# evfro/polara

Measured on NVIDIA H100. Metric: user-item pairs scored/sec (fused top-k) at rank 50, higher is better.
Workload: dtype f32 (bf16 tensor-core filter, exact fp32 rescoring)

## Files before the change

polara_b200/csrc/topk_tc.cu:

```cuda
#include <cuda_bf16.h>
#include <cstdlib>
#include <cub/device/device_radix_sort.cuh>

#include "topk_common.cuh"

namespace {

constexpr int BM = 128;
constexpr int BN = 128;
constexpr int NCONS = 256;
constexpr int NTHREADS = NCONS + 32;
constexpr int CAPS = 16;
constexpr int MAX_STAGES = 10;
constexpr uint32_t STAGE_BYTES = BN * 128;
constexpr int PROBE_ITEMS = 256;
constexpr int HEAD_TILES = 8;
constexpr int HEAD_WORDS = HEAD_TILES * BN / 32;
constexpr long long SPIN_LIMIT_CYCLES = 4000000000ll;

struct TcParams {
    const __nv_bfloat16* Ap;
    const __nv_bfloat16* Bp;
    const float* E; int64_t lde;
    const float* V; int64_t ldv;
// ... 106 lines not shown

__device__ __forceinline__ uint32_t bf16_floor_bits(float x) {
    uint32_t b = __float_as_uint(x);
    uint32_t hi = b >> 16;
    if ((b & 0xFFFFu) && (b >> 31)) hi += 1;
    return hi;
}
__device__ __forceinline__ uint32_t bf16_ceil_pos_bits(float x) {
    uint32_t b = __float_as_uint(x);
    return (b >> 16) + ((b & 0xFFFFu) ? 1u : 0u);
}
__device__ __forceinline__ uint32_t pack_threshold(float t) {
    if (!(t > -3.0e38f)) t = -3.0e38f;
    t -= fabsf(t) * 1.52587890625e-5f;
    uint32_t hi = bf16_floor_bits(t);
    float hif = __uint_as_float(hi << 16);
    float rem = t - hif;
    uint32_t lo = bf16_floor_bits(rem);
    return (lo << 16) | (hi & 0xFFFFu);
}

__global__ void pack_items_kernel(const float* __restrict__ V, int64_t ldv, int64_t n, int r, int rs, int KP,
                                  int64_t item_tiles, const int32_t* __restrict__ perm,
                                  const float* __restrict__ vnorm_sorted, __nv_bfloat16* __restrict__ Bp) {
    const int chunks = (KP + 63) / 64 * 8;
    int64_t gid = (int64_t)blockIdx.x * blockDim.x + threadIdx.x;
    int64_t total = item_tiles * BN * chunks;
    if (gid >= total) return;
    int64_t tile = gid / ((int64_t)BN * chunks);
    int rem = (int)(gid % ((int64_t)BN * chunks));
    int row = rem / chunks, ch = rem % chunks;
    int64_t pos = tile * BN + row;
    const int64_t item = pos < n ? (int64_t)__ldg(perm + pos) : -1;
    __align__(16) __nv_bfloat16 out[8];
#pragma unroll
    for (int j = 0; j < 8; ++j) {
        int kk = ch * 8 + j;
        float x = 0.f;
        if (item >= 0) {
            if (kk < r) x = __ldg(V + item * ldv + kk);
            else if (kk == rs || kk == rs + 1) x = 1.0f;
        }
        out[j] = __float2bfloat16_rn(x);
        if (item >= 0 && kk == rs + 2) out[j] = __ushort_as_bfloat16((unsigned short)bf16_ceil_pos_bits(__ldg(vnorm_sorted + pos)));
    }
    size_t byte = (size_t)tile * BN * chunks * 16 + tile_byte(BN, row, ch * 8);
    *reinterpret_cast<uint4*>(reinterpret_cast<unsigned char*>(Bp) + byte) = *reinterpret_cast<const uint4*>(out);
}

__global__ void pack_users_kernel(const float* __restrict__ E, int64_t lde, int64_t m, int r, int rs, int KP,
                                  int64_t user_tiles, const int32_t* __restrict__ uperm, const float* __restrict__ enorm,
                                  const float* __restrict__ t0, __nv_bfloat16* __restrict__ Ap) {
    const int chunks = (KP + 63) / 64 * 8;
    int64_t gid = (int64_t)blockIdx.x * blockDim.x + threadIdx.x;
    int64_t total = user_tiles * BM * chunks;
    if (gid >= total) return;
    int64_t tile = gid / ((int64_t)BM * chunks);
    int rem = (int)(gid % ((int64_t)BM * chunks));
    int row = rem / chunks, ch = rem % chunks;
    const int64_t tr = tile * BM + row;
    const int64_t u = (tr < m && uperm) ? (int64_t)__ldg(uperm + tr) : tr;
    __align__(16) __nv_bfloat16 out[8];
    uint32_t thr = 0;
    if (ch == rs / 8) {
        if (u < m) {
            thr = pack_threshold(t0[u]);
        } else {
            thr = 0x00007F7Fu;
        }
    }
#pragma unroll
    for (int j = 0; j < 8; ++j) {
        int kk = ch * 8 + j;
        float x = 0.f;
        if (u < m && kk < r) x = -__ldg(E + u * lde + kk);
        out[j] = __float2bfloat16_rn(x);
        if (kk == rs) out[j] = __ushort_as_bfloat16((unsigned short)(thr & 0xFFFFu));
        if (kk == rs + 1) out[j] = __ushort_as_bfloat16((unsigned short)(thr >> 16));
        if (kk == rs + 2 && u < m)
            out[j] = __ushort_as_bfloat16((unsigned short)(0x8000u | bf16_ceil_pos_bits(0.0079345703125f * enorm[u] + 1e-30f)));
    }
    size_t byte = (size_t)tile * BM * chunks * 16 + tile_byte(BM, row, ch * 8);
    *reinterpret_cast<uint4*>(reinterpret_cast<unsigned char*>(Ap) + byte) = *reinterpret_cast<const uint4*>(out);
}

__global__ void row_norm_kernel(const float* __restrict__ X, int64_t ld, int64_t rows, int r, float* __restrict__ norms,
                                float* __restrict__ max_out) {
    int64_t w = ((int64_t)blockIdx.x * blockDim.x + threadIdx.x) >> 5;
    int lane = threadIdx.x & 31;
    if (w >= rows) return;
    float s = 0.f;
    for (int t = lane; t < r; t += 32) { float x = __ldg(X + w * ld + t); s = fmaf(x, x, s); }
#pragma unroll
    for (int o = 16; o > 0; o >>= 1) s += __shfl_xor_sync(0xffffffffu, s, o);
    s = sqrtf(s) * 1.0001f;
    if (lane == 0) {
        if (norms) norms[w] = s;
        if (max_out) atomicMax(reinterpret_cast<int*>(max_out), __float_as_int(s));
    }
}

__global__ void iota_i32_kernel(int32_t* __restrict__ x, int64_t n) {
    int64_t i = (int64_t)blockIdx.x * blockDim.x + threadIdx.x;
    if (i < n) x[i] = (int32_t)i;
}

__global__ void invert_perm_kernel(const int32_t* __restrict__ perm, int64_t n, int32_t* __restrict__ inv) {
    int64_t i = (int64_t)blockIdx.x * blockDim.x + threadIdx.x;
    if (i < n) inv[perm[i]] = (int32_t)i;
}

__global__ void head_items_kernel(const int32_t* __restrict__ perm, int64_t n_head, uint32_t* __restrict__ in_head) {
    int64_t i = (int64_t)blockIdx.x * blockDim.x + threadIdx.x;
    if (i < n_head) { const int32_t item = perm[i]; atomicOr(in_head + (item >> 5), 1u << (item & 31)); }
}

__global__ void __launch_bounds__(256)
head_bitmap_kernel(const int64_t* __restrict__ seen_indptr, const int32_t* __restrict__ seen_indices,
                   int64_t seen_offset, const int32_t* __restrict__ inv_perm, const uint32_t* __restrict__ in_head,
                   int64_t m, int64_t n, uint32_t* __restrict__ bits) {
    static_assert(HEAD_WORDS == 32, "one bitmap word per lane");
    __shared__ uint32_t sw[8][HEAD_WORDS];
    const int64_t u = ((int64_t)blockIdx.x * blockDim.x + threadIdx.x) >> 5;
    const int lane = threadIdx.x & 31, warp = threadIdx.x >> 5;
    if (u >= m) return;
    sw[warp][lane] = 0u;
    __syncwarp();
    for (int64_t p = seen_indptr[u] + lane; p < seen_indptr[u + 1]; p += 32) {
        int64_t item = (int64_t)__ldg(seen_indices + p) - seen_offset;
        if (item < 0 || item >= n) continue;
        if (!((__ldg(in_head + (item >> 5)) >> (item & 31)) & 1u)) continue;
        int pos = __ldg(inv_perm + item);
        atomicOr(&sw[warp][pos >> 5], 0x80000000u >> (pos & 31));
    }
    __syncwarp();
    bits[u * HEAD_WORDS + lane] = sw[warp][lane];
}

__device__ __forceinline__ int first_cut_tile(float en, float t, const float* __restrict__ vnorm_sorted, int lo, int hi) {
    if (!(t > 0.f && t < CUDART_INF_F)) return hi;
    while (lo < hi) {
        const int mid = (lo + hi) >> 1;
        if (en * __ldg(vnorm_sorted + (int64_t)mid * BN) < t) hi = mid; else lo = mid + 1;
    }
    return lo;
}

__global__ void user_need_kernel(const float* __restrict__ enorm, const float* __restrict__ t0,
                                 const float* __restrict__ vnorm_sorted, int64_t m, int item_tiles, int32_t* __restrict__ need) {
    const int64_t u = (int64_t)blockIdx.x * blockDim.x + threadIdx.x;
    if (u < m) need[u] = first_cut_tile(__ldg(enorm + u), __ldg(t0 + u), vnorm_sorted, 0, item_tiles);
}

constexpr int PTU = 64, PTI = 128, PKS = 32;
constexpr int PNU = 2;
template <int PI>
struct ProbeSmem {
    float es[PKS][PTU + 4];
    float vs[PKS][PTI + 4];
    float sc[PTU][PI + 4];
    unsigned long long cand[8][PNU][32];
    float t0s[PTU];
};

__device__ __forceinline__ uint32_t ord_of(float x) {
    const uint32_t b = __float_as_uint(x);
    return (b & 0x80000000u) ? ~b : (b | 0x80000000u);
}
__device__ __forceinline__ float ord_to_float(uint32_t o) {
    return __uint_as_float((o & 0x80000000u) ? (o & 0x7FFFFFFFu) : ~o);
}

template <int PL>
__device__ __noinline__ void probe_select_rounds(unsigned long long (&key)[PL], int lane, int k,
                                                 pb200_cand* __restrict__ out, float* __restrict__ t0_u) {
    static_assert(PL == 8, "the sorting network below is for 8 keys per lane");
#define PB_CAS(A, B) { const unsigned long long x_ = key[A], y_ = key[B]; const bool g_ = x_ > y_; key[A] = g_ ? x_ : y_; key[B] = g_ ? y_ : x_; }
    PB_CAS(0, 1) PB_CAS(2, 3) PB_CAS(4, 5) PB_CAS(6, 7)
    PB_CAS(0, 2) PB_CAS(1, 3) PB_CAS(4, 6) PB_CAS(5, 7)
    PB_CAS(1, 2) PB_CAS(5, 6)
    PB_CAS(0, 4) PB_CAS(1, 5) PB_CAS(2, 6) PB_CAS(3, 7)
    PB_CAS(2, 4) PB_CAS(3, 5)
    PB_CAS(1, 2) PB_CAS(3, 4) PB_CAS(5, 6)
#undef PB_CAS
    float kth = -CUDART_INF_F;
    int produced = 0;
    pb200_cand mine; mine.score = -CUDART_INF_F; mine.id = -1;
    for (; produced < k; ++produced) {
        const uint32_t hh = (uint32_t)(key[0] >> 32), hl = (uint32_t)key[0];
        const uint32_t wh = __reduce_max_sync(0xffffffffu, hh);
        if (wh == 0u) break;
        const uint32_t wl = __reduce_max_sync(0xffffffffu, hh == wh ? hl : 0u);
        if (hh == wh && hl == wl) {
#pragma unroll
            for (int j = 0; j + 1 < PL; ++j) key[j] = key[j + 1];
            key[PL - 1] = 0ull;
        }
        const float ws = ord_to_float(wh);
        if (lane == (produced & 31)) { mine.score = ws; mine.id = (int)(0xFFFFFFFFu - wl); }
        if ((produced & 31) == 31) out[(produced - 31) + lane] = mine;
        kth = ws;
    }
    if (lane < (produced & 31)) out[(produced & ~31) + lane] = mine;
    for (int j = produced + lane; j < k; j += 32) { pb200_cand c; c.score = -CUDART_INF_F; c.id = -1; out[j] = c; }
    if (lane == 0) *t0_u = produced == k ? kth : -CUDART_INF_F;
}

template <int PI>
__global__ void __launch_bounds__(256)
probe_kernel(const float* __restrict__ E, int64_t lde, const float* __restrict__ V, int64_t ldv,
             const int32_t* __restrict__ perm, int64_t m, int64_t n_probe, int r, int k,
             const uint32_t* __restrict__ headbits, float* __restrict__ t0, pb200_cand* __restrict__ out_list,
             float* __restrict__ enorm, const float* __restrict__ vnorm_sorted, int item_tiles, int32_t* __restrict__ need) {
    extern __shared__ __align__(16) unsigned char praw[];
    ProbeSmem<PI>& sm = *reinterpret_cast<ProbeSmem<PI>*>(praw);
    const int tid = threadIdx.x, lane = tid & 31, warp = tid >> 5, tx = tid & 15, ty = tid >> 4;
    const int64_t u0 = (int64_t)blockIdx.x * PTU;
    const bool vec = ((lde | ldv) & 3) == 0 && ((reinterpret_cast<uintptr_t>(E) | reinterpret_cast<uintptr_t>(V)) & 15) == 0;
    const int n_ktiles = (r + PKS - 1) / PKS, n_tiles = (PI / PTI) * n_ktiles;
    const int64_t eu = u0 + (tid & (PTU - 1));
    const float* erow = eu < m ? E + eu * lde : nullptr;
    const float* vrow = nullptr;
    float4 pe[2], pv[4];
    auto fetch = [&](int tile) {
        const int i0 = (tile / n_ktiles) * PTI, k0 = (tile % n_ktiles) * PKS;
        if (tile % n_ktiles == 0) {
            const int64_t vpos = i0 + (tid & (PTI - 1));
            vrow = vpos < n_probe ? V + (int64_t)__ldg(perm + vpos) * ldv : nullptr;
        }
#pragma unroll
        for (int it = 0; it < 2; ++it) {
            const int kq = k0 + 4 * ((tid >> 6) + 4 * it);
            pe[it] = (erow && kq < r) ? __ldg(reinterpret_cast<const float4*>(erow + kq)) : make_float4(0.f, 0.f, 0.f, 0.f);
        }
#pragma unroll
        for (int it = 0; it < 4; ++it) {
            const int kq = k0 + 4 * ((tid >> 7) + 2 * it);
            pv[it] = (vrow && kq < r) ? __ldg(reinterpret_cast<const float4*>(vrow + kq)) : make_float4(0.f, 0.f, 0.f, 0.f);
        }
    };
    auto stash = [&](int tile) {
        const int k0 = (tile % n_ktiles) * PKS;
#pragma unroll
        for (int it = 0; it < 2; ++it) {
            const int q = (tid >> 6) + 4 * it, kq = k0 + 4 * q, row = tid & (PTU - 1);
            sm.es[4 * q + 0][row] = pe[it].x;
            sm.es[4 * q + 1][row] = kq + 1 < r ? pe[it].y : 0.f;
            sm.es[4 * q + 2][row] = kq + 2 < r ? pe[it].z : 0.f;
            sm.es[4 * q + 3][row] = kq + 3 < r ? pe[it].w : 0.f;
        }
#pragma unroll
        for (int it = 0; it < 4; ++it) {
            const int q = (tid >> 7) + 2 * it, kq = k0 + 4 * q, row = tid & (PTI - 1);
            sm.vs[4 * q + 0][row] = pv[it].x;
            sm.vs[4 * q + 1][row] = kq + 1 < r ? pv[it].y : 0.f;
            sm.vs[4 * q + 2][row] = kq + 2 < r ? pv[it].z : 0.f;
            sm.vs[4 * q + 3][row] = kq + 3 < r ? pv[it].w : 0.f;
        }
    };
    if (vec) fetch(0);
    float acc[4][8];
    float en2 = 0.f;
    for (int tile = 0; tile < n_tiles; ++tile) {
        const int i0 = (tile / n_ktiles) * PTI, k0 = (tile % n_ktiles) * PKS;
        if (k0 == 0) {
#pragma unroll
            for (int a = 0; a < 4; ++a)
#pragma unroll
                for (int b = 0; b < 8; ++b) acc[a][b] = 0.f;
        }
        if (vec) {
            stash(tile);
        } else {
#pragma unroll
            for (int it = 0; it < 8; ++it) {
                int e = tid + it * 256, row = e >> 5, kk = e & 31;
                int64_t u = u0 + row;
                sm.es[kk][row] = (u < m && k0 + kk < r) ? __ldg(E + u * lde + k0 + kk) : 0.f;
            }
#pragma unroll
            for (int it = 0; it < 16; ++it) {
                int e = tid + it * 256, row = e >> 5, kk = e & 31;
                int64_t pos = i0 + row;
                sm.vs[kk][row] = (pos < n_probe && k0 + kk < r) ? __ldg(V + (int64_t)__ldg(perm + pos) * ldv + k0 + kk) : 0.f;
            }
        }
        __syncthreads();
        if (vec && tile + 1 < n_tiles) fetch(tile + 1);
        const int kmax = min(PKS, r - k0);
        if (i0 == 0 && tid < PTU)
            for (int kk = 0; kk < kmax; ++kk) en2 = fmaf(sm.es[kk][tid], sm.es[kk][tid], en2);
        for (int kk = 0; kk < kmax; ++kk) {
            float4 e4 = *reinterpret_cast<const float4*>(&sm.es[kk][ty * 4]);
            float4 v0 = *reinterpret_cast<const float4*>(&sm.vs[kk][tx * 4]);
            float4 v1 = *reinterpret_cast<const float4*>(&sm.vs[kk][64 + tx * 4]);
            float a[4] = {e4.x, e4.y, e4.z, e4.w};
            float b[8] = {v0.x, v0.y, v0.z, v0.w, v1.x, v1.y, v1.z, v1.w};
#pragma unroll
            for (int i = 0; i < 4; ++i)
#pragma unroll
                for (int j = 0; j < 8; ++j) acc[i][j] = fmaf(a[i], b[j], acc[i][j]);
        }
        if (k0 + PKS >= r) {
#pragma unroll
            for (int i = 0; i < 4; ++i)
#pragma unroll
                for (int hseg = 0; hseg < 2; ++hseg) {
                    const int pos = i0 + 64 * hseg + tx * 4;
                    float4 x;
                    x.x = pos + 0 < n_probe ? acc[i][4 * hseg + 0] : -CUDART_INF_F;
                    x.y = pos + 1 < n_probe ? acc[i][4 * hseg + 1] : -CUDART_INF_F;
                    x.z = pos + 2 < n_probe ? acc[i][4 * hseg + 2] : -CUDART_INF_F;
                    x.w = pos + 3 < n_probe ? acc[i][4 * hseg + 3] : -CUDART_INF_F;
                    *reinterpret_cast<float4*>(&sm.sc[ty * 4 + i][pos]) = x;
                }
        }
        __syncthreads();
    }
    constexpr int PL = PI / 32;
    const uint32_t lt_mask = (1u << lane) - 1u;
    for (int ul = warp; ul < PTU; ul += 8 * PNU) {
        int64_t u[PNU];
        bool act[PNU];
        uint32_t seen_w[PNU], ord[PNU][PL], lmax[PNU], tau[PNU];
        int count[PNU] = {};
#pragma unroll
        for (int a = 0; a < PNU; ++a) {
            u[a] = u0 + ul + 8 * a;
            act[a] = ul + 8 * a < PTU && u[a] < m;
            seen_w[a] = 0u;
            if (act[a] && headbits && lane < PL) seen_w[a] = __ldg(headbits + u[a] * HEAD_WORDS + lane);
        }
#pragma unroll
        for (int a = 0; a < PNU; ++a) {
            lmax[a] = 0u;
#pragma unroll
            for (int j = 0; j < PL; ++j) {
                const int pos = lane + 32 * j;
                const uint32_t w = __shfl_sync(0xffffffffu, seen_w[a], j);
                const bool ok = act[a] && pos < n_probe && !(w & (0x80000000u >> lane));
                ord[a][j] = ok ? ord_of(sm.sc[act[a] ? ul + 8 * a : 0][pos]) : 0u;
                lmax[a] = max(lmax[a], ord[a][j]);
            }
        }
        const bool small_k = k <= 32;
        if (small_k) {
            uint32_t rest[PNU], w[PNU];
#pragma unroll
            for (int a = 0; a < PNU; ++a) { rest[a] = lmax[a]; w[a] = 0u; }
            for (int i = 0; i < k; ++i) {
#pragma unroll
                for (int a = 0; a < PNU; ++a) {
                    w[a] = __reduce_max_sync(0xffffffffu, rest[a]);
                    if (rest[a] == w[a]) rest[a] = 0u;
                }
            }
#pragma unroll
            for (int a = 0; a < PNU; ++a) tau[a] = w[a] == 0u ? 1u : w[a];
#pragma unroll
            for (int a = 0; a < PNU; ++a) count[a] = 0;
#pragma unroll
            for (int j = 0; j < PL; ++j)
#pragma unroll
                for (int a = 0; a < PNU; ++a) {
                    const bool in = ord[a][j] >= tau[a];
                    const uint32_t b = __ballot_sync(0xffffffffu, in);
                    const int slot = count[a] + __popc(b & lt_mask);
                    if (in && slot < 32) sm.cand[warp][a][slot] = ((unsigned long long)ord[a][j] << 32) | (uint32_t)(lane + 32 * j);
                    count[a] += __popc(b);
                }
        }
        bool fast[PNU];
#pragma unroll
        for (int a = 0; a < PNU; ++a) fast[a] = act[a] && small_k && count[a] <= 32;
        __syncwarp();
        unsigned long long mine[PNU];
#pragma unroll
        for (int a = 0; a < PNU; ++a) {
            mine[a] = 0ull;
            if (fast[a] && lane < count[a]) {
                const unsigned long long c = sm.cand[warp][a][lane];
                const uint32_t id = (uint32_t)__ldg(perm + (uint32_t)c);
                mine[a] = (c & 0xFFFFFFFF00000000ull) | (unsigned long long)(0xFFFFFFFFu - id);
            }
        }
        __syncwarp();
#pragma unroll
        for (int a = 0; a < PNU; ++a) if (fast[a]) sm.cand[warp][a][lane] = mine[a];
        __syncwarp();
#pragma unroll
        for (int a = 0; a < PNU; ++a) {
            if (!fast[a]) continue;
            pb200_cand* out = out_list + u[a] * k;
            int rank = 0;
            for (int t = 0; t < count[a]; ++t) rank += sm.cand[warp][a][t] > mine[a] ? 1 : 0;
            if (lane < count[a] && rank < k) {
                pb200_cand c; c.score = ord_to_float((uint32_t)(mine[a] >> 32)); c.id = (int)(0xFFFFFFFFu - (uint32_t)mine[a]);
                out[rank] = c;
                if (rank == k - 1) sm.t0s[ul + 8 * a] = c.score;
            }
            if (count[a] < k) {
                if (lane >= count[a] && lane < k) { pb200_cand c; c.score = -CUDART_INF_F; c.id = -1; out[lane] = c; }
                if (lane == 0) sm.t0s[ul + 8 * a] = -CUDART_INF_F;
            }
        }
        __syncwarp();
#pragma unroll
        for (int a = 0; a < PNU; ++a) {
            if (!act[a] || fast[a]) continue;
            unsigned long long key[PL];
#pragma unroll
            for (int j = 0; j < PL; ++j) {
                const uint32_t id = ord[a][j] ? (uint32_t)__ldg(perm + lane + 32 * j) : 0u;
                key[j] = ord[a][j] ? (((unsigned long long)ord[a][j] << 32) | (unsigned long long)(0xFFFFFFFFu - id)) : 0ull;
            }
            probe_select_rounds<PL>(key, lane, k, out_list + u[a] * k, &sm.t0s[ul + 8 * a]);
        }
    }
    __syncthreads();
    if (tid < PTU && u0 + tid < m) {
        const int64_t uu = u0 + tid;
        const float t = sm.t0s[tid], en = sqrtf(en2) * 1.0001f;
        t0[uu] = t;
        enorm[uu] = en;
        if (need) need[uu] = first_cut_tile(en, t, vnorm_sorted, 0, item_tiles);
    }
}

__device__ __forceinline__ float exact_score_vec(const float* __restrict__ erow, const float* __restrict__ vrow, int r, bool vec_ok) {
    if (!vec_ok) return exact_score(erow, vrow, r);
    const int r4 = r / 4;
    const float4* e4 = reinterpret_cast<const float4*>(erow);
    const float4* v4 = reinterpret_cast<const float4*>(vrow);
    float s = 0.f;
    int t = 0;
    for (; t + 8 <= r4; t += 8) {
        float4 a[8], b[8];
#pragma unroll
        for (int i = 0; i < 8; ++i) { a[i] = __ldg(e4 + t + i); b[i] = __ldg(v4 + t + i); }
#pragma unroll
        for (int i = 0; i < 8; ++i) {
            s = fmaf(a[i].x, b[i].x, s); s = fmaf(a[i].y, b[i].y, s);
            s = fmaf(a[i].z, b[i].z, s); s = fmaf(a[i].w, b[i].w, s);
        }
    }
    for (; t + 4 <= r4; t += 4) {
        float4 a[4], b[4];
#pragma unroll
        for (int i = 0; i < 4; ++i) { a[i] = __ldg(e4 + t + i); b[i] = __ldg(v4 + t + i); }
#pragma unroll
        for (int i = 0; i < 4; ++i) {
            s = fmaf(a[i].x, b[i].x, s); s = fmaf(a[i].y, b[i].y, s);
            s = fmaf(a[i].z, b[i].z, s); s = fmaf(a[i].w, b[i].w, s);
        }
    }
    for (; t < r4; ++t) {
        float4 a = __ldg(e4 + t), b = __ldg(v4 + t);
        s = fmaf(a.x, b.x, s); s = fmaf(a.y, b.y, s); s = fmaf(a.z, b.z, s); s = fmaf(a.w, b.w, s);
    }
    for (int tt = r4 * 4; tt < r; ++tt) s = fmaf(__ldg(erow + tt), __ldg(vrow + tt), s);
    return s;
}

struct ListState {
    pb200_cand* list;
    int cnt;
    float kth;
};

__device__ __forceinline__ void list_insert(ListState& ls, int k, float s, int id) {
    if (ls.cnt == k) {
        pb200_cand last = ls.list[k - 1];
        if (!cand_before(s, id, last.score, last.id)) return;
    }
    int i = ls.cnt < k ? ls.cnt : k - 1;
    while (i > 0) {
        pb200_cand p = ls.list[i - 1];
        if (!cand_before(s, id, p.score, p.id)) break;
        ls.list[i] = p;
        --i;
    }
    pb200_cand c; c.score = s; c.id = id;
    ls.list[i] = c;
    if (ls.cnt < k) ls.cnt++;
    if (ls.cnt == k) ls.kth = ls.list[k - 1].score;
}

constexpr int COOP_MIN = 64;
struct CoopArgs {
    const float* V; int64_t ldv; const int32_t* perm; const int32_t* seen_indices; int64_t seen_offset; int64_t n; int r, k;
};
__device__ __noinline__ int coop_flush_row(const CoopArgs p, const float* __restrict__ erow, const uint2* __restrict__ stage_row,
                                           int n_entries, int64_t t_lo, int64_t sb, int64_t se, bool head_masked,
                                           pb200_cand* __restrict__ list, float t_row, bool vec_ok, int lane, int& cnt, float& kth) {
    int n_scored = 0;
    for (int e = 0; e < n_entries; ++e) {
        const uint2 ent = stage_row[e * 256];
        const int64_t pos = (int64_t)(t_lo + (ent.x >> 2)) * BN + (ent.x & 3) * 32 + lane;
        bool ok = ((ent.y << lane) & 0x80000000u) != 0u && pos < p.n;
        int item = -1;
        float s = 0.f;
        if (ok) {
            item = __ldg(p.perm + pos);
            if (sb < se && (!head_masked || pos >= HEAD_TILES * BN) &&
                seen_lookup(p.seen_indices, sb, se, (int)(item + p.seen_offset))) ok = false;
        }
        if (ok) {
            s = exact_score_vec(erow, p.V + (int64_t)item * p.ldv, p.r, vec_ok);
            ++n_scored;
            ok = !(s < t_row);
        }
        uint32_t pass = __ballot_sync(0xffffffffu, ok);
        while (pass) {
            const int l = __ffs(pass) - 1;
            pass &= pass - 1;
            const float sl = __shfl_sync(0xffffffffu, s, l);
            const int il = __shfl_sync(0xffffffffu, item, l);
            if (sl < t_row) continue;
            cnt = warp_list_insert(list, p.k, cnt, sl, il, lane);
            if (cnt == p.k) { kth = list[p.k - 1].score; t_row = fmaxf(t_row, kth); }
        }
    }
    return n_scored;
}

__global__ void __launch_bounds__(NTHREADS, 1)
score_topk_tc_kernel(const TcParams p) {
    extern __shared__ __align__(1024) unsigned char smem[];
    unsigned char* sA = smem + ((1024u - (smem_u32(smem) & 1023u)) & 1023u);
    unsigned char* sB = sA + p.a_bytes;
    uint2* sStage = reinterpret_cast<uint2*>(sB + (size_t)p.stages * STAGE_BYTES);
    volatile uint2* sThr = reinterpret_cast<volatile uint2*>(sStage + CAPS * 256);
    uint64_t* bars = reinterpret_cast<uint64_t*>(const_cast<uint2*>(sThr) + 256);
    const uint32_t bar_full = smem_u32(bars), bar_empty = smem_u32(bars + MAX_STAGES);
    const uint32_t bar_afull = smem_u32(bars + 2 * MAX_STAGES), bar_aempty = smem_u32(bars + 2 * MAX_STAGES + 1);
    volatile uint32_t* flush_gen = reinterpret_cast<volatile uint32_t*>(bars + 2 * MAX_STAGES + 2);
    volatile unsigned long long* sCut = reinterpret_cast<volatile unsigned long long*>(bars + 2 * MAX_STAGES + 4);
    volatile uint32_t* sStop = reinterpret_cast<volatile uint32_t*>(bars + 2 * MAX_STAGES + 4 + NCONS / 32);

    const int tid = threadIdx.x, warp = tid >> 5, lane = tid & 31;
    if (tid < 256) { const_cast<uint2*>(sThr)[tid] = make_uint2(0u, 0u); }
    if (tid < NCONS / 32) sCut[tid] = 0ull;
    if (tid < MAX_STAGES) sStop[tid] = 0u;
    if (tid == 0) {
        *flush_gen = 0u;
        for (int s = 0; s < p.stages; ++s) { mbar_init(bar_full + 8 * s, 1); mbar_init(bar_empty + 8 * s, NCONS / 32); }
        mbar_init(bar_afull, 1);
        mbar_init(bar_aempty, NCONS / 32);
        fence_barrier_init();
        if (p.hdbg && blockIdx.x == 0) p.hdbg[5] = bar_full;
    }
    __syncthreads();

    const int64_t n_groups = p.user_tiles * p.parts;
    const int64_t n_ctas = gridDim.x, cta = blockIdx.x;
    WorkItem wk;
    const uint32_t S = (uint32_t)p.stages;
    const int KA = (p.KP + 63) / 64;

    if (warp == NCONS / 32) {
        if (lane == 0) {
            uint32_t stage = 0, phase = 0, awork = 0;
            for (int64_t wi = 0; next_work(p, wi, cta, n_ctas, n_groups, wk); ++wi, ++awork) {
                const int64_t t_lo = min(p.item_tiles, p.tile_first + (int64_t)wk.part * p.tiles_per_part);
                int64_t t_hi = min(p.item_tiles, p.tile_first + (int64_t)(wk.part + 1) * p.tiles_per_part);
                if (p.need_sorted) t_hi = min(t_hi, max(t_lo, (int64_t)__ldg(p.need_sorted + wk.g * BM)));
                mbar_wait(bar_aempty, (awork & 1) ^ 1, p.stats, p.hdbg);
                mbar_arrive_expect_tx(bar_afull, p.a_bytes);
                bulk_g2s(smem_u32(sA), reinterpret_cast<const unsigned char*>(p.Ap) + (size_t)wk.g * p.a_bytes, p.a_bytes, bar_afull);
                for (int64_t t = t_lo; t < t_hi; ++t) {
                    if (p.need_sorted) {
                        bool all = true;
                        int64_t live_cut = 0;
#pragma unroll
                        for (int w = 0; w < NCONS / 32; ++w) {
                            const unsigned long long e = sCut[w];
                            all = all && (uint32_t)e == awork + 1;
                            live_cut = max(live_cut, (int64_t)(e >> 32));
// ... 133 lines not shown
                const int64_t t = t_lo + j;
                if (p.need_sorted) {
                    const uint32_t st = gslab % S, ph = (gslab / S) & 1u;
                    mbar_wait(bar_full + 8 * st, ph, p.stats, p.hdbg);
                    if (sStop[st]) {
                        ++gslab;
                        __syncwarp();
                        if (lane == 0) mbar_arrive(bar_empty + 8 * st);
                        break;
                    }
                }
                float d[64];
#pragma unroll
                for (int i = 0; i < 64; ++i) d[i] = 0.f;
                uint32_t prev = 0;
                for (int sl = 0; sl < KA; ++sl) {
                    const uint32_t st = gslab % S, ph = (gslab / S) & 1u;
                    ++gslab;
                    mbar_wait(bar_full + 8 * st, ph, p.stats, p.hdbg);
                    wg_fence_acc(d);
                    wg_fence();
#pragma unroll
                    for (int ks = 0; ks < 4; ++ks)
                        wgmma_m64n128k16(d, adesc0 + (uint64_t)((uint32_t)sl * (BM * 128 / 16) + (uint32_t)ks * 2),
                                         bdesc0 + (uint64_t)(st * (STAGE_BYTES / 16) + (uint32_t)ks * 2), (sl | ks) != 0);
                    wg_commit();
                    wg_fence_acc(d);
                    if (sl > 0) {
                        wg_wait<1>();
                        __syncwarp();
                        if (lane == 0) mbar_arrive(bar_empty + 8 * prev);
                    }
                    prev = st;
                }
                wg_wait<0>();
                wg_fence_acc(d);
                __syncwarp();
                if (lane == 0) mbar_arrive(bar_empty + 8 * prev);

                uint32_t w[2][4];
#pragma unroll
                for (int a = 0; a < 2; ++a)
#pragma unroll
                    for (int c = 0; c < 4; ++c) {
                        uint32_t mk = 0;
#pragma unroll
                        for (int i = 0; i < 4; ++i)
#pragma unroll
                            for (int b = 0; b < 2; ++b)
                                mk |= (__float_as_uint(d[4 * (4 * c + i) + 2 * a + b]) >> 31) << (31 - 8 * i - b);
                        mk >>= 2 * q;
                        mk |= __shfl_xor_sync(0xffffffffu, mk, 1);
                        mk |= __shfl_xor_sync(0xffffffffu, mk, 2);
                        w[a][c] = mk;
                    }
                const bool hi_row = (q >> 1) != 0;
                uint32_t m0 = hi_row ? (h ? w[1][2] : w[1][0]) : (h ? w[0][2] : w[0][0]);
                uint32_t m1 = hi_row ? (h ? w[1][3] : w[1][1]) : (h ? w[0][3] : w[0][1]);
                if (head && t < HEAD_TILES) {
                    const uint2 hb = __ldg(reinterpret_cast<const uint2*>(head + (int)t * (BN / 32) + 2 * h));
                    m0 &= ~hb.x; m1 &= ~hb.y;
                }
                const uint32_t code = (uint32_t)j << 2;
                if (m0 && live) { sStage[scount * 256 + etid] = make_uint2(code | (uint32_t)(2 * h), m0); ++scount; }
                if (m1 && live) { sStage[scount * 256 + etid] = make_uint2(code | (uint32_t)(2 * h + 1), m1); ++scount; }
                {
                    const uint32_t gen = *flush_gen;
                    const bool need = __any_sync(0xffffffffu, scount > CAPS - 2 || (scount >= 4 && t_row == -CUDART_INF_F));
                    if (need || gen != my_gen) {
                        if (need && gen == my_gen && lane == 0) atomicAdd(const_cast<uint32_t*>(flush_gen), 1u);
                        flush();
                        my_gen = *flush_gen;
                        if (p.need_sorted) publish_cut(t + 1);
                    }
                }
            }
            n_swept += (unsigned long long)j;
            flush();
            __syncwarp();
            if (lane == 0) mbar_arrive(bar_aempty);
        }
        if (p.stats && n_rescored) atomicAdd(p.stats + 1, n_rescored);
        if (p.stats && tid == 0 && n_swept) atomicAdd(p.stats + 5, n_swept);
    }
    __syncthreads();
}

}

int pb_score_tc(pb200_ctx* ctx, const float* E, int64_t lde, const float* V, int64_t ldv, int64_t m, int64_t n,
                int r, const int64_t* seen_indptr, const int32_t* seen_indices, int64_t seen_offset, int k,
                int* parts_out, pb200_cand** lists_out, Scratch& sc) {
    const int rs = (r + 1) & ~1;
    const int KP = ((rs + 3) + 15) / 16 * 16;
    const int KA = (KP + 63) / 64;
    const uint32_t a_bytes = BM * KA * 128, b_bytes = BN * KA * 128;
    const size_t fixed = (size_t)a_bytes + CAPS * 256 * sizeof(uint2) + 256 * sizeof(uint2) + (2 * MAX_STAGES + 4) * 8 +
                         (NCONS / 32) * 8 + MAX_STAGES * 4 + 1024;
    int dev_smem = 0;
    PB_CUDA(ctx, cudaDeviceGetAttribute(&dev_smem, cudaDevAttrMaxSharedMemoryPerBlockOptin, ctx->device));
    const int64_t user_tiles = ceil_div64(m, BM), item_tiles = ceil_div64(n, BN);
    const int stages = (int)std::min<int64_t>(MAX_STAGES, ((int64_t)dev_smem - (int64_t)fixed) / STAGE_BYTES);
    if (stages < 2) {
        ctx->err = "tensor-core scoring kernel: rank too large for the shared-memory pipeline (use the simt kernel)";
        return PB200_ENOTIMPL;
    }
    const int64_t n_probe = std::min<int64_t>(PROBE_ITEMS, (n / BN) * BN);
    const int64_t tile_first = n_probe / BN, sweep_tiles = item_tiles - tile_first;
    int parts = (int)std::max<int64_t>(1, std::min<int64_t>(std::min<int64_t>(ceil_div64(2 * (int64_t)ctx->num_sms, user_tiles), 64),
                                                              std::max<int64_t>(sweep_tiles, 1)));
    const int64_t tiles_per_part = std::max<int64_t>(1, ceil_div64(sweep_tiles, parts));
    parts = (int)std::max<int64_t>(1, ceil_div64(sweep_tiles, tiles_per_part));

    __nv_bfloat16 *Ap = nullptr, *Bp = nullptr;
    float *enorm = nullptr, *vnorm = nullptr, *vnorm_sorted = nullptr, *t0 = nullptr;
    int32_t *iota = nullptr, *perm = nullptr, *inv_perm = nullptr;
    uint32_t* headbits = nullptr;
    pb200_cand* lists = nullptr;
    PB_TRY(sc.alloc(&Ap, (size_t)user_tiles * BM * KA * 64));
    PB_TRY(sc.alloc(&Bp, (size_t)item_tiles * BN * KA * 64));
    PB_TRY(sc.alloc(&enorm, (size_t)m));
    PB_TRY(sc.alloc(&vnorm, (size_t)n));
    PB_TRY(sc.alloc(&vnorm_sorted, (size_t)n));
    PB_TRY(sc.alloc(&iota, (size_t)n));
    PB_TRY(sc.alloc(&perm, (size_t)n));
    PB_TRY(sc.alloc(&t0, (size_t)m));
    PB_TRY(sc.alloc(&lists, (size_t)(parts * 2 + 1) * m * k));

    row_norm_kernel<<<(unsigned)ceil_div64(n * 32, 256), 256, 0, ctx->stream>>>(V, ldv, n, r, vnorm, nullptr);
    iota_i32_kernel<<<(unsigned)ceil_div64(n, 256), 256, 0, ctx->stream>>>(iota, n);
    {
        size_t temp_bytes = 0;
        PB_CUDA(ctx, cub::DeviceRadixSort::SortPairsDescending(nullptr, temp_bytes, vnorm, vnorm_sorted, iota, perm, (int64_t)n, 0, 32, ctx->stream));
        uint8_t* temp = nullptr;
        PB_TRY(sc.alloc(&temp, temp_bytes));
        PB_CUDA(ctx, cub::DeviceRadixSort::SortPairsDescending(temp, temp_bytes, vnorm, vnorm_sorted, iota, perm, (int64_t)n, 0, 32, ctx->stream));
    }
    if (seen_indptr) {
        PB_TRY(sc.alloc(&inv_perm, (size_t)n));
        PB_TRY(sc.alloc(&headbits, (size_t)m * HEAD_WORDS));
        invert_perm_kernel<<<(unsigned)ceil_div64(n, 256), 256, 0, ctx->stream>>>(perm, n, inv_perm);
        uint32_t* in_head = nullptr;
        const int64_t n_head = std::min<int64_t>(n, (int64_t)HEAD_TILES * BN);
        PB_TRY(sc.alloc(&in_head, (size_t)ceil_div64(n, 32)));
        PB_CUDA(ctx, cudaMemsetAsync(in_head, 0, (size_t)ceil_div64(n, 32) * sizeof(uint32_t), ctx->stream));
        head_items_kernel<<<(unsigned)ceil_div64(n_head, 256), 256, 0, ctx->stream>>>(perm, n_head, in_head);
        head_bitmap_kernel<<<(unsigned)ceil_div64(m * 32, 256), 256, 0, ctx->stream>>>(seen_indptr, seen_indices, seen_offset,
                                                                                     inv_perm, in_head, m, n, headbits);
    }
    const bool prune = ctx->prune != 0;
    int32_t* need = nullptr;
    if (prune) PB_TRY(sc.alloc(&need, (size_t)m));
    {
        PB_CUDA(ctx, cudaFuncSetAttribute(probe_kernel<PROBE_ITEMS>, cudaFuncAttributeMaxDynamicSharedMemorySize, (int)sizeof(ProbeSmem<PROBE_ITEMS>)));
        probe_kernel<PROBE_ITEMS><<<(unsigned)ceil_div64(m, PTU), 256, sizeof(ProbeSmem<PROBE_ITEMS>), ctx->stream>>>(
            E, lde, V, ldv, perm, m, n_probe, r, k, headbits, t0, lists + (size_t)parts * 2 * m * k,
            enorm, vnorm_sorted, (int)item_tiles, ctx->bound_fn ? nullptr : need);
    }
    if (ctx->bound_fn) {
        const int st = ctx->bound_fn(ctx->bound_user, t0, m, PB200_F32);
        if (st != 0) {
            ctx->err = "bound hook failed with status " + std::to_string(st);
            return PB200_ECUDA;
        }
        if (prune) user_need_kernel<<<(unsigned)ceil_div64(m, 256), 256, 0, ctx->stream>>>(enorm, t0, vnorm_sorted, m, (int)item_tiles, need);
    }
    int32_t *uperm = nullptr, *need_sorted = nullptr;
    if (prune) {
        int32_t* uiota = nullptr;
        PB_TRY(sc.alloc(&uiota, (size_t)m));
        PB_TRY(sc.alloc(&uperm, (size_t)m));
        PB_TRY(sc.alloc(&need_sorted, (size_t)m));
        iota_i32_kernel<<<(unsigned)ceil_div64(m, 256), 256, 0, ctx->stream>>>(uiota, m);
        int end_bit = 1;
        while (end_bit < 31 && ((int64_t)1 << end_bit) <= item_tiles) ++end_bit;
        size_t temp_bytes = 0;
        PB_CUDA(ctx, cub::DeviceRadixSort::SortPairsDescending(nullptr, temp_bytes, need, need_sorted, uiota, uperm, m, 0, end_bit, ctx->stream));
        uint8_t* temp = nullptr;
        PB_TRY(sc.alloc(&temp, temp_bytes));
        PB_CUDA(ctx, cub::DeviceRadixSort::SortPairsDescending(temp, temp_bytes, need, need_sorted, uiota, uperm, m, 0, end_bit, ctx->stream));
    }
    {
        int64_t tot_b = item_tiles * BN * (KA * 8), tot_a = user_tiles * BM * (KA * 8);
        pack_items_kernel<<<(unsigned)ceil_div64(tot_b, 256), 256, 0, ctx->stream>>>(V, ldv, n, r, rs, KP, item_tiles, perm, vnorm_sorted, Bp);
        pack_users_kernel<<<(unsigned)ceil_div64(tot_a, 256), 256, 0, ctx->stream>>>(E, lde, m, r, rs, KP, user_tiles, uperm, enorm, t0, Ap);
    }
    if (sweep_tiles <= 0) {
        cudaEventRecord(ctx->ev0, ctx->stream);
        cudaEventRecord(ctx->ev1, ctx->stream);
        *parts_out = 1;
        *lists_out = lists + (size_t)parts * 2 * m * k;
        PB_CUDA(ctx, cudaGetLastError());
        return PB200_OK;
    }
    TcParams p;
    p.Ap = Ap; p.Bp = Bp; p.E = E; p.lde = lde; p.V = V; p.ldv = ldv; p.perm = perm; p.t0 = t0;
    p.m = m; p.n = n; p.r = r; p.KP = KP; p.rs = rs; p.k = k;
    p.user_tiles = user_tiles; p.item_tiles = item_tiles; p.parts = parts; p.tiles_per_part = tiles_per_part;
    p.tile_first = tile_first;
    p.seen_indptr = seen_indptr; p.seen_indices = seen_indices; p.seen_offset = seen_offset;
    p.lists = lists; p.stages = stages; p.a_bytes = a_bytes; p.b_bytes = b_bytes;
    p.uperm = uperm; p.need_sorted = need_sorted; p.enorm = enorm; p.vnorm_sorted = vnorm_sorted; p.headbits = headbits;
    p.stats = reinterpret_cast<unsigned long long*>(ctx->d_stats);
    p.hdbg = nullptr;
    if (ctx->h_dbg) {
        unsigned long long* dptr = nullptr;
        if (cudaHostGetDevicePointer(&dptr, ctx->h_dbg, 0) == cudaSuccess) p.hdbg = dptr;
    }
    const size_t smem_bytes = fixed + (size_t)stages * STAGE_BYTES;
    PB_CUDA(ctx, cudaFuncSetAttribute(score_topk_tc_kernel, cudaFuncAttributeMaxDynamicSharedMemorySize, (int)smem_bytes));
    const int64_t n_groups = user_tiles * parts;
    const unsigned grid = (unsigned)std::min<int64_t>(n_groups, ctx->num_sms);
    cudaEventRecord(ctx->ev0, ctx->stream);
    score_topk_tc_kernel<<<grid, NTHREADS, smem_bytes, ctx->stream>>>(p);
    cudaEventRecord(ctx->ev1, ctx->stream);
    ctx->stats[0] += (seen_indptr ? 13 : 10) + (prune ? 2 : 0) + (prune && ctx->bound_fn ? 1 : 0);
    ctx->stats[2] = (uint64_t)item_tiles; ctx->stats[3] = (uint64_t)user_tiles;
    ctx->stats[6] += (uint64_t)(user_tiles * sweep_tiles);
    PB_CUDA(ctx, cudaGetLastError());
    *parts_out = parts * 2 + 1;
    *lists_out = lists;
    return PB200_OK;
}
```

Before: 15500 billion.

## Restructure probe kernel as persistent per-warp user batches with resident item slab

The probe kernel is rewritten so each warp handles batches of 8 users. The 256 probe item vectors stay resident in shared memory across batches when rank fits in one slab, so V is no longer reloaded for every 64-user tile. Scores stay in registers instead of going through a shared score matrix. Seen-item bitmaps arrive via cp.async, and a persistent grid sized from occupancy strides over the batches. This cuts redundant V traffic and block-wide syncs, but per-warp work is serialized and register pressure rises with the 8x8 accumulator.

```diff
diff --git a/polara_b200/csrc/topk_tc.cu b/polara_b200/csrc/topk_tc.cu
--- a/polara_b200/csrc/topk_tc.cu
+++ b/polara_b200/csrc/topk_tc.cu
@@ -282,15 +282,17 @@
     if (u < m) need[u] = first_cut_tile(__ldg(enorm + u), __ldg(t0 + u), vnorm_sorted, 0, item_tiles);
 }
 
-constexpr int PTU = 64, PTI = 128, PKS = 32;
+constexpr int PKS = 64;
+constexpr int PB = 8;
+constexpr int PW = 8;
 constexpr int PNU = 2;
-template <int PI>
 struct ProbeSmem {
-    float es[PKS][PTU + 4];
-    float vs[PKS][PTI + 4];
-    float sc[PTU][PI + 4];
-    unsigned long long cand[8][PNU][32];
-    float t0s[PTU];
+    float vs[PKS][PROBE_ITEMS];
+    float es[PW][PKS][PB];
+    unsigned long long cand[PW][PNU][32];
+    float t0s[PW][PB];
+    int32_t ids[PROBE_ITEMS];
+    uint32_t bits[PW][PB][8];
 };
 
 __device__ __forceinline__ uint32_t ord_of(float x) {
@@ -336,224 +338,217 @@
     if (lane == 0) *t0_u = produced == k ? kth : -CUDART_INF_F;
 }
 
-template <int PI>
-__global__ void __launch_bounds__(256)
+__device__ __forceinline__ float4 probe_quad(const float* __restrict__ row, int kq, int r, bool vec) {
+    float4 x = make_float4(0.f, 0.f, 0.f, 0.f);
+    if (row == nullptr || kq >= r) return x;
+    if (vec) {
+        x = __ldg(reinterpret_cast<const float4*>(row + kq));
+        if (kq + 1 >= r) x.y = 0.f;
+        if (kq + 2 >= r) x.z = 0.f;
+        if (kq + 3 >= r) x.w = 0.f;
+    } else {
+        x.x = __ldg(row + kq);
+        if (kq + 1 < r) x.y = __ldg(row + kq + 1);
+        if (kq + 2 < r) x.z = __ldg(row + kq + 2);
+        if (kq + 3 < r) x.w = __ldg(row + kq + 3);
+    }
+    return x;
+}
+
+__device__ __forceinline__ void cp_async4(void* dst, const void* src) {
+    asm volatile("cp.async.ca.shared.global [%0], [%1], 4;" ::"r"(smem_u32(dst)), "l"(src) : "memory");
+}
+__device__ __forceinline__ void cp_async_wait_all() { asm volatile("cp.async.wait_all;" ::: "memory"); }
+
+__device__ __forceinline__ int probe_pos(int lane, int j) { return (j < 4 ? 0 : 128) + 4 * lane + (j & 3); }
+
+__global__ void __launch_bounds__(PW * 32, 2)
 probe_kernel(const float* __restrict__ E, int64_t lde, const float* __restrict__ V, int64_t ldv,
              const int32_t* __restrict__ perm, int64_t m, int64_t n_probe, int r, int k,
              const uint32_t* __restrict__ headbits, float* __restrict__ t0, pb200_cand* __restrict__ out_list,
              float* __restrict__ enorm, const float* __restrict__ vnorm_sorted, int item_tiles, int32_t* __restrict__ need) {
+    static_assert(PROBE_ITEMS == 256 && PB == 8, "lane l owns positions 4 l + {0..3, 128..131} of 8 users");
     extern __shared__ __align__(16) unsigned char praw[];
-    ProbeSmem<PI>& sm = *reinterpret_cast<ProbeSmem<PI>*>(praw);
-    const int tid = threadIdx.x, lane = tid & 31, warp = tid >> 5, tx = tid & 15, ty = tid >> 4;
-    const int64_t u0 = (int64_t)blockIdx.x * PTU;
+    ProbeSmem& sm = *reinterpret_cast<ProbeSmem*>(praw);
+    const int tid = threadIdx.x, lane = tid & 31, warp = tid >> 5;
+    float (&es)[PKS][PB] = sm.es[warp];
     const bool vec = ((lde | ldv) & 3) == 0 && ((reinterpret_cast<uintptr_t>(E) | reinterpret_cast<uintptr_t>(V)) & 15) == 0;
-    const int n_ktiles = (r + PKS - 1) / PKS, n_tiles = (PI / PTI) * n_ktiles;
-    const int64_t eu = u0 + (tid & (PTU - 1));
-    const float* erow = eu < m ? E + eu * lde : nullptr;
-    const float* vrow = nullptr;
-    float4 pe[2], pv[4];
-    auto fetch = [&](int tile) {
-        const int i0 = (tile / n_ktiles) * PTI, k0 = (tile % n_ktiles) * PKS;
-        if (tile % n_ktiles == 0) {
-            const int64_t vpos = i0 + (tid & (PTI - 1));
-            vrow = vpos < n_probe ? V + (int64_t)__ldg(perm + vpos) * ldv : nullptr;
-        }
-#pragma unroll
-        for (int it = 0; it < 2; ++it) {
-            const int kq = k0 + 4 * ((tid >> 6) + 4 * it);
-            pe[it] = (erow && kq < r) ? __ldg(reinterpret_cast<const float4*>(erow + kq)) : make_float4(0.f, 0.f, 0.f, 0.f);
-        }
-#pragma unroll
-        for (int it = 0; it < 4; ++it) {
-            const int kq = k0 + 4 * ((tid >> 7) + 2 * it);
-            pv[it] = (vrow && kq < r) ? __ldg(reinterpret_cast<const float4*>(vrow + kq)) : make_float4(0.f, 0.f, 0.f, 0.f);
-        }
+    const int n_slabs = (r + PKS - 1) / PKS;
+    const int64_t n_batches = (m + PB - 1) / PB, first = (int64_t)blockIdx.x * PW, stride = (int64_t)gridDim.x * PW;
+
+    float4 pe[4];
+    auto fetch_e = [&](int64_t b, int s) {
+        const int64_t u = b * PB + (lane & 7);
+        const float* erow = u < m ? E + u * lde : nullptr;
+#pragma unroll
+        for (int i = 0; i < 4; ++i) pe[i] = probe_quad(erow, s * PKS + 4 * ((lane >> 3) + 4 * i), r, vec);
     };
-    auto stash = [&](int tile) {
-        const int k0 = (tile % n_ktiles) * PKS;
-#pragma unroll
-        for (int it = 0; it < 2; ++it) {
-            const int q = (tid >> 6) + 4 * it, kq = k0 + 4 * q, row = tid & (PTU - 1);
-            sm.es[4 * q + 0][row] = pe[it].x;
-            sm.es[4 * q + 1][row] = kq + 1 < r ? pe[it].y : 0.f;
-            sm.es[4 * q + 2][row] = kq + 2 < r ? pe[it].z : 0.f;
-            sm.es[4 * q + 3][row] = kq + 3 < r ? pe[it].w : 0.f;
-        }
-#pragma unroll
-        for (int it = 0; it < 4; ++it) {
-            const int q = (tid >> 7) + 2 * it, kq = k0 + 4 * q, row = tid & (PTI - 1);
-            sm.vs[4 * q + 0][row] = pv[it].x;
-            sm.vs[4 * q + 1][row] = kq + 1 < r ? pv[it].y : 0.f;
-            sm.vs[4 * q + 2][row] = kq + 2 < r ? pv[it].z : 0.f;
-            sm.vs[4 * q + 3][row] = kq + 3 < r ? pv[it].w : 0.f;
-        }
-    };
-    if (vec) fetch(0);
-    float acc[4][8];
+    fetch_e(first + warp, 0);
+    const uint32_t lt_mask = (1u << lane) - 1u;
     float en2 = 0.f;
-    for (int tile = 0; tile < n_tiles; ++tile) {
-        const int i0 = (tile / n_ktiles) * PTI, k0 = (tile % n_ktiles) * PKS;
-        if (k0 == 0) {
-#pragma unroll
-            for (int a = 0; a < 4; ++a)
-#pragma unroll
-                for (int b = 0; b < 8; ++b) acc[a][b] = 0.f;
-        }
-        if (vec) {
-            stash(tile);
-        } else {
-#pragma unroll
-            for (int it = 0; it < 8; ++it) {
-                int e = tid + it * 256, row = e >> 5, kk = e & 31;
-                int64_t u = u0 + row;
-                sm.es[kk][row] = (u < m && k0 + kk < r) ? __ldg(E + u * lde + k0 + kk) : 0.f;
-            }
-#pragma unroll
-            for (int it = 0; it < 16; ++it) {
-                int e = tid + it * 256, row = e >> 5, kk = e & 31;
-                int64_t pos = i0 + row;
-                sm.vs[kk][row] = (pos < n_probe && k0 + kk < r) ? __ldg(V + (int64_t)__ldg(perm + pos) * ldv + k0 + kk) : 0.f;
-            }
-        }
-        __syncthreads();
-        if (vec && tile + 1 < n_tiles) fetch(tile + 1);
-        const int kmax = min(PKS, r - k0);
-        if (i0 == 0 && tid < PTU)
-            for (int kk = 0; kk < kmax; ++kk) en2 = fmaf(sm.es[kk][tid], sm.es[kk][tid], en2);
-        for (int kk = 0; kk < kmax; ++kk) {
-            float4 e4 = *reinterpret_cast<const float4*>(&sm.es[kk][ty * 4]);
-            float4 v0 = *reinterpret_cast<const float4*>(&sm.vs[kk][tx * 4]);
-            float4 v1 = *reinterpret_cast<const float4*>(&sm.vs[kk][64 + tx * 4]);
-            float a[4] = {e4.x, e4.y, e4.z, e4.w};
-            float b[8] = {v0.x, v0.y, v0.z, v0.w, v1.x, v1.y, v1.z, v1.w};
-#pragma unroll
-            for (int i = 0; i < 4; ++i)
-#pragma unroll
-                for (int j = 0; j < 8; ++j) acc[i][j] = fmaf(a[i], b[j], acc[i][j]);
-        }
-        if (k0 + PKS >= r) {
-#pragma unroll
-            for (int i = 0; i < 4; ++i)
-#pragma unroll
-                for (int hseg = 0; hseg < 2; ++hseg) {
-                    const int pos = i0 + 64 * hseg + tx * 4;
-                    float4 x;
-                    x.x = pos + 0 < n_probe ? acc[i][4 * hseg + 0] : -CUDART_INF_F;
-                    x.y = pos + 1 < n_probe ? acc[i][4 * hseg + 1] : -CUDART_INF_F;
-                    x.z = pos + 2 < n_probe ? acc[i][4 * hseg + 2] : -CUDART_INF_F;
-                    x.w = pos + 3 < n_probe ? acc[i][4 * hseg + 3] : -CUDART_INF_F;
-                    *reinterpret_cast<float4*>(&sm.sc[ty * 4 + i][pos]) = x;
-                }
-        }
-        __syncthreads();
-    }
-    constexpr int PL = PI / 32;
-    const uint32_t lt_mask = (1u << lane) - 1u;
-    for (int ul = warp; ul < PTU; ul += 8 * PNU) {
-        int64_t u[PNU];
-        bool act[PNU];
-        uint32_t seen_w[PNU], ord[PNU][PL], lmax[PNU], tau[PNU];
-        int count[PNU] = {};
-#pragma unroll
-        for (int a = 0; a < PNU; ++a) {
-            u[a] = u0 + ul + 8 * a;
-            act[a] = ul + 8 * a < PTU && u[a] < m;
-            seen_w[a] = 0u;
-            if (act[a] && headbits && lane < PL) seen_w[a] = __ldg(headbits + u[a] * HEAD_WORDS + lane);
-        }
-#pragma unroll
-        for (int a = 0; a < PNU; ++a) {
-            lmax[a] = 0u;
-#pragma unroll
-            for (int j = 0; j < PL; ++j) {
-                const int pos = lane + 32 * j;
-                const uint32_t w = __shfl_sync(0xffffffffu, seen_w[a], j);
-                const bool ok = act[a] && pos < n_probe && !(w & (0x80000000u >> lane));
-                ord[a][j] = ok ? ord_of(sm.sc[act[a] ? ul + 8 * a : 0][pos]) : 0u;
-                lmax[a] = max(lmax[a], ord[a][j]);
-            }
-        }
-        const bool small_k = k <= 32;
-        if (small_k) {
-            uint32_t rest[PNU], w[PNU];
-#pragma unroll
-            for (int a = 0; a < PNU; ++a) { rest[a] = lmax[a]; w[a] = 0u; }
-            for (int i = 0; i < k; ++i) {
-#pragma unroll
-                for (int a = 0; a < PNU; ++a) {
-                    w[a] = __reduce_max_sync(0xffffffffu, rest[a]);
-                    if (rest[a] == w[a]) rest[a] = 0u;
-                }
-            }
-#pragma unroll
-            for (int a = 0; a < PNU; ++a) tau[a] = w[a] == 0u ? 1u : w[a];
-#pragma unroll
-            for (int a = 0; a < PNU; ++a) count[a] = 0;
-#pragma unroll
-            for (int j = 0; j < PL; ++j)
-#pragma unroll
-                for (int a = 0; a < PNU; ++a) {
-                    const bool in = ord[a][j] >= tau[a];
-                    const uint32_t b = __ballot_sync(0xffffffffu, in);
-                    const int slot = count[a] + __popc(b & lt_mask);
-                    if (in && slot < 32) sm.cand[warp][a][slot] = ((unsigned long long)ord[a][j] << 32) | (uint32_t)(lane + 32 * j);
-                    count[a] += __popc(b);
-                }
-        }
-        bool fast[PNU];
-#pragma unroll
-        for (int a = 0; a < PNU; ++a) fast[a] = act[a] && small_k && count[a] <= 32;
+    for (int64_t base = first; base < n_batches; base += stride) {
+        const int64_t b = base + warp;
+        float acc[PB][8];
+#pragma unroll
+        for (int i = 0; i < PB; ++i)
+#pragma unroll
+            for (int j = 0; j < 8; ++j) acc[i][j] = 0.f;
+        for (int s = 0; s < n_slabs; ++s) {
+            __syncwarp();
+#pragma unroll
+            for (int i = 0; i < 4; ++i) {
+                const int q = (lane >> 3) + 4 * i, u = lane & 7;
+                es[4 * q + 0][u] = pe[i].x; es[4 * q + 1][u] = pe[i].y; es[4 * q + 2][u] = pe[i].z; es[4 * q + 3][u] = pe[i].w;
+            }
+            if (n_slabs > 1 || base == first) {
+                __syncthreads();
+                const int32_t item = tid < n_probe ? __ldg(perm + tid) : 0;
+                const float* vrow = tid < n_probe ? V + (int64_t)item * ldv : nullptr;
+                if (s == 0) sm.ids[tid] = item;
+#pragma unroll 4
+                for (int q = 0; q < PKS / 4; ++q) {
+                    const float4 x = probe_quad(vrow, s * PKS + 4 * q, r, vec);
+                    sm.vs[4 * q + 0][tid] = x.x; sm.vs[4 * q + 1][tid] = x.y; sm.vs[4 * q + 2][tid] = x.z; sm.vs[4 * q + 3][tid] = x.w;
+                }
+                __syncthreads();
+            } else {
+                __syncwarp();
+            }
+            if (s + 1 < n_slabs) fetch_e(b, s + 1); else fetch_e(b + stride, 0);
+            if (s == 0) {
+#pragma unroll
+                for (int i = 0; i < 2; ++i) {
+                    const int w = lane + 32 * i, ul = w >> 3;
+                    const int64_t u = b * PB + ul;
+                    if (headbits && u < m) cp_async4(&sm.bits[warp][ul][w & 7], headbits + u * HEAD_WORDS + (w & 7));
+                    else sm.bits[warp][ul][w & 7] = 0u;
+                }
+            }
+            const int kmax = min(PKS, r - s * PKS);
+            if (lane < PB)
+                for (int kk = 0; kk < kmax; ++kk) en2 = fmaf(es[kk][lane], es[kk][lane], en2);
+#pragma unroll 1
+            for (int kk = 0; kk < kmax; ++kk) {
+                const float4 e0 = *reinterpret_cast<const float4*>(&es[kk][0]);
+                const float4 e1 = *reinterpret_cast<const float4*>(&es[kk][4]);
+                const float4 v0 = *reinterpret_cast<const float4*>(&sm.vs[kk][4 * lane]);
+                const float4 v1 = *reinterpret_cast<const float4*>(&sm.vs[kk][128 + 4 * lane]);
+                const float e[PB] = {e0.x, e0.y, e0.z, e0.w, e1.x, e1.y, e1.z, e1.w};
+                const float v[8] = {v0.x, v0.y, v0.z, v0.w, v1.x, v1.y, v1.z, v1.w};
+#pragma unroll
+                for (int i = 0; i < PB; ++i)
+#pragma unroll
+                    for (int j = 0; j < 8; ++j) acc[i][j] = fmaf(e[i], v[j], acc[i][j]);
+            }
+        }
+        const uint32_t sh = 31u - 4u * (uint32_t)(lane & 7);
+        cp_async_wait_all();
         __syncwarp();
-        unsigned long long mine[PNU];
-#pragma unroll
-        for (int a = 0; a < PNU; ++a) {
-            mine[a] = 0ull;
-            if (fast[a] && lane < count[a]) {
-                const unsigned long long c = sm.cand[warp][a][lane];
-                const uint32_t id = (uint32_t)__ldg(perm + (uint32_t)c);
-                mine[a] = (c & 0xFFFFFFFF00000000ull) | (unsigned long long)(0xFFFFFFFFu - id);
-            }
+#pragma unroll 1
+        for (int ub = 0; ub < PB; ub += PNU) {
+            int64_t u[PNU];
+            bool act[PNU];
+            uint32_t ord[PNU][8], lmax[PNU], tau[PNU];
+            int count[PNU] = {};
+#pragma unroll
+            for (int a = 0; a < PNU; ++a) {
+                u[a] = b * PB + ub + a;
+                act[a] = u[a] < m;
+                const uint32_t w0 = sm.bits[warp][ub + a][lane >> 3], w1 = sm.bits[warp][ub + a][4 + (lane >> 3)];
+                lmax[a] = 0u;
+#pragma unroll
+                for (int j = 0; j < 8; ++j) {
+                    const uint32_t w = j < 4 ? w0 : w1;
+                    const bool ok = act[a] && probe_pos(lane, j) < n_probe && !((w >> (sh - (j & 3))) & 1u);
+                    ord[a][j] = ok ? ord_of(acc[a][j]) : 0u;
+                    lmax[a] = max(lmax[a], ord[a][j]);
+                }
+            }
+            const bool small_k = k <= 32;
+            if (small_k) {
+                uint32_t rest[PNU], w[PNU];
+#pragma unroll
+                for (int a = 0; a < PNU; ++a) { rest[a] = lmax[a]; w[a] = 0u; }
+                for (int i = 0; i < k; ++i) {
+#pragma unroll
+                    for (int a = 0; a < PNU; ++a) {
+                        w[a] = __reduce_max_sync(0xffffffffu, rest[a]);
+                        if (rest[a] == w[a]) rest[a] = 0u;
+                    }
+                }
+#pragma unroll
+                for (int a = 0; a < PNU; ++a) tau[a] = w[a] == 0u ? 1u : w[a];
+#pragma unroll
+                for (int j = 0; j < 8; ++j)
+#pragma unroll
+                    for (int a = 0; a < PNU; ++a) {
+                        const bool in = ord[a][j] >= tau[a];
+                        const uint32_t bal = __ballot_sync(0xffffffffu, in);
+                        const int slot = count[a] + __popc(bal & lt_mask);
+                        if (in && slot < 32) sm.cand[warp][a][slot] = ((unsigned long long)ord[a][j] << 32) | (uint32_t)probe_pos(lane, j);
+                        count[a] += __popc(bal);
+                    }
+            }
+            bool fast[PNU];
+#pragma unroll
+            for (int a = 0; a < PNU; ++a) fast[a] = act[a] && small_k && count[a] <= 32;
+            __syncwarp();
+            unsigned long long mine[PNU];
+#pragma unroll
+            for (int a = 0; a < PNU; ++a) {
+                mine[a] = 0ull;
+                if (fast[a] && lane < count[a]) {
+                    const unsigned long long c = sm.cand[warp][a][lane];
+                    const uint32_t id = (uint32_t)sm.ids[(uint32_t)c];
+                    mine[a] = (c & 0xFFFFFFFF00000000ull) | (unsigned long long)(0xFFFFFFFFu - id);
+                }
+            }
+            __syncwarp();
+#pragma unroll
+            for (int a = 0; a < PNU; ++a) if (fast[a]) sm.cand[warp][a][lane] = mine[a];
+            __syncwarp();
+#pragma unroll
+            for (int a = 0; a < PNU; ++a) {
+                if (!fast[a]) continue;
+                pb200_cand* out = out_list + u[a] * k;
+                int rank = 0;
+                for (int t = 0; t < count[a]; ++t) rank += sm.cand[warp][a][t] > mine[a] ? 1 : 0;
+                if (lane < count[a] && rank < k) {
+                    pb200_cand c; c.score = ord_to_float((uint32_t)(mine[a] >> 32)); c.id = (int)(0xFFFFFFFFu - (uint32_t)mine[a]);
+                    out[rank] = c;
+                    if (rank == k - 1) sm.t0s[warp][ub + a] = c.score;
+                }
+                if (count[a] < k) {
+                    if (lane >= count[a] && lane < k) { pb200_cand c; c.score = -CUDART_INF_F; c.id = -1; out[lane] = c; }
+                    if (lane == 0) sm.t0s[warp][ub + a] = -CUDART_INF_F;
+                }
+            }
+            __syncwarp();
+#pragma unroll
+            for (int a = 0; a < PNU; ++a) {
+                if (!act[a] || fast[a]) continue;
+                unsigned long long key[8];
+#pragma unroll
+                for (int j = 0; j < 8; ++j) {
+                    const uint32_t id = ord[a][j] ? (uint32_t)sm.ids[probe_pos(lane, j)] : 0u;
+                    key[j] = ord[a][j] ? (((unsigned long long)ord[a][j] << 32) | (unsigned long long)(0xFFFFFFFFu - id)) : 0ull;
+                }
+                probe_select_rounds<8>(key, lane, k, out_list + u[a] * k, &sm.t0s[warp][ub + a]);
+            }
+#pragma unroll
+            for (int i = 0; i + PNU < PB; ++i)
+#pragma unroll
+                for (int j = 0; j < 8; ++j) acc[i][j] = acc[i + PNU][j];
         }
         __syncwarp();
-#pragma unroll
-        for (int a = 0; a < PNU; ++a) if (fast[a]) sm.cand[warp][a][lane] = mine[a];
-        __syncwarp();
-#pragma unroll
-        for (int a = 0; a < PNU; ++a) {
-            if (!fast[a]) continue;
-            pb200_cand* out = out_list + u[a] * k;
-            int rank = 0;
-            for (int t = 0; t < count[a]; ++t) rank += sm.cand[warp][a][t] > mine[a] ? 1 : 0;
-            if (lane < count[a] && rank < k) {
-                pb200_cand c; c.score = ord_to_float((uint32_t)(mine[a] >> 32)); c.id = (int)(0xFFFFFFFFu - (uint32_t)mine[a]);
-                out[rank] = c;
-                if (rank == k - 1) sm.t0s[ul + 8 * a] = c.score;
-            }
-            if (count[a] < k) {
-                if (lane >= count[a] && lane < k) { pb200_cand c; c.score = -CUDART_INF_F; c.id = -1; out[lane] = c; }
-                if (lane == 0) sm.t0s[ul + 8 * a] = -CUDART_INF_F;
-            }
-        }
-        __syncwarp();
-#pragma unroll
-        for (int a = 0; a < PNU; ++a) {
-            if (!act[a] || fast[a]) continue;
-            unsigned long long key[PL];
-#pragma unroll
-            for (int j = 0; j < PL; ++j) {
-                const uint32_t id = ord[a][j] ? (uint32_t)__ldg(perm + lane + 32 * j) : 0u;
-                key[j] = ord[a][j] ? (((unsigned long long)ord[a][j] << 32) | (unsigned long long)(0xFFFFFFFFu - id)) : 0ull;
-            }
-            probe_select_rounds<PL>(key, lane, k, out_list + u[a] * k, &sm.t0s[ul + 8 * a]);
-        }
-    }
-    __syncthreads();
-    if (tid < PTU && u0 + tid < m) {
-        const int64_t uu = u0 + tid;
-        const float t = sm.t0s[tid], en = sqrtf(en2) * 1.0001f;
-        t0[uu] = t;
-        enorm[uu] = en;
-        if (need) need[uu] = first_cut_tile(en, t, vnorm_sorted, 0, item_tiles);
+        if (lane < PB && b * PB + lane < m) {
+            const int64_t uu = b * PB + lane;
+            const float t = sm.t0s[warp][lane], en = sqrtf(en2) * 1.0001f;
+            t0[uu] = t;
+            enorm[uu] = en;
+            if (need) need[uu] = first_cut_tile(en, t, vnorm_sorted, 0, item_tiles);
+        }
+        en2 = 0.f;
     }
 }
 
@@ -993,8 +988,12 @@
     int32_t* need = nullptr;
     if (prune) PB_TRY(sc.alloc(&need, (size_t)m));
     {
-        PB_CUDA(ctx, cudaFuncSetAttribute(probe_kernel<PROBE_ITEMS>, cudaFuncAttributeMaxDynamicSharedMemorySize, (int)sizeof(ProbeSmem<PROBE_ITEMS>)));
-        probe_kernel<PROBE_ITEMS><<<(unsigned)ceil_div64(m, PTU), 256, sizeof(ProbeSmem<PROBE_ITEMS>), ctx->stream>>>(
+        PB_CUDA(ctx, cudaFuncSetAttribute(probe_kernel, cudaFuncAttributeMaxDynamicSharedMemorySize, (int)sizeof(ProbeSmem)));
+        int per_sm = 0;
+        PB_CUDA(ctx, cudaOccupancyMaxActiveBlocksPerMultiprocessor(&per_sm, probe_kernel, PW * 32, sizeof(ProbeSmem)));
+        const int64_t rounds = ceil_div64(ceil_div64(m, PB), PW);
+        const unsigned grid = (unsigned)std::max<int64_t>(1, std::min<int64_t>(rounds, (int64_t)std::max(per_sm, 1) * ctx->num_sms));
+        probe_kernel<<<grid, PW * 32, sizeof(ProbeSmem), ctx->stream>>>(
             E, lde, V, ldv, perm, m, n_probe, r, k, headbits, t0, lists + (size_t)parts * 2 * m * k,
             enorm, vnorm_sorted, (int)item_tiles, ctx->bound_fn ? nullptr : need);
     }
```

New measurement: 16070 billion, median of 6. 3.7% higher.
